# hlesmqh/WS3D

Hardware: AMD Instinct MI355X
Metric: KITTI scenes/sec (16384 pts) Stage-1 RPN fwd, 1/2/4/8 GPU; FPS+group HBM GB/s (higher is better)
Workload: dtype f32

## Files before the change

include/ws3d_ops.h:

```cpp
#ifndef WS3D_OPS_H
#define WS3D_OPS_H

#include <stddef.h>
#include <stdint.h>

#ifdef __cplusplus
extern "C" {
#endif

#define WS3D_OK 0
#define WS3D_E_INVALID (-1)
#define WS3D_E_LAUNCH (-2)
#define WS3D_E_WORKSPACE (-3)
#define WS3D_E_UNSUPPORTED (-4)

#if defined(__GNUC__)
#define WS3D_API __attribute__((visibility("default")))
#else
#define WS3D_API
#endif

typedef void *ws3d_stream_t;

#define WS3D_ABI_VERSION 6
// ... 162 lines not shown
                                const int32_t *idx, const float *weight, float *grad_points,
                                ws3d_stream_t stream);

WS3D_API size_t ws3d_scatter_workspace_bytes(int b, int c, int n_targets, long slots_per_scene);
WS3D_API int ws3d_group_points_grad_det(int b, int c, int n, int npoints, int nsample, const float *grad_out,
                                        const int32_t *idx, float *grad_points, void *workspace,
                                        size_t workspace_bytes, ws3d_stream_t stream);
WS3D_API int ws3d_three_interpolate_grad_det(int b, int c, int n, int m, const float *grad_out, const int32_t *idx,
                                             const float *weight, float *grad_points, void *workspace,
                                             size_t workspace_bytes, ws3d_stream_t stream);

WS3D_API int ws3d_bias_act_inplace(int b, int o_ch, long l, int relu, float *y, const float *bias,
                                   ws3d_stream_t stream);

WS3D_API int ws3d_rowmax_bias_act(int b, int o_ch, long m, int s, int relu, const float *y, const float *bias,
                                  float *out, ws3d_stream_t stream);

WS3D_API int ws3d_query_and_group_nlc(int b, int n, int m, int c, float radius, int nsample, int use_xyz,
                                      const float *xyz, const float *new_xyz, const float *features_nlc,
                                      int32_t *idx_out, float *out_nlc, const void *sorted, ws3d_stream_t stream);
WS3D_API int ws3d_three_interpolate_nlc(int b, int c, int m, int n, const float *feats_nlc, const int32_t *idx,
                                        const float *weight, float *out_nlc, int out_stride, ws3d_stream_t stream);
WS3D_API int ws3d_rowmax_rows(long rows_out, int ns, int o_ch, const float *y, float *out, int out_stride,
                              ws3d_stream_t stream);

WS3D_API int ws3d_sa_mlp3_pool(long rows, int nsample, int c1, int c2, int c3, const float *x_rows4,
                               const float *w1t, const float *b1, const float *w2t, const float *b2,
                               const float *w3t, const float *b3, int relu3, float *out, int out_stride,
                               ws3d_stream_t stream);

WS3D_API int ws3d_mlp2_rows(long rows, int k_dim, int o1, int o2, const float *x_rows, const float *w1t, const float *b1, int relu1,
                   const float *w2t, const float *b2, int relu2, float *out, int *ticket, ws3d_stream_t stream);

WS3D_API int ws3d_qinterp_gemm(int b, int n, int m, int c, int o_dim, const float *q, const int32_t *idx, const float *weight, const float *lin,
                      const float *skip, int c1, const float *wb, const float *b1, int relu1, const float *w2t, const float *b2, int relu2,
                      float *out, ws3d_stream_t stream);


WS3D_API int ws3d_boxes_overlap_bev(int num_a, const float *boxes_a, int num_b, const float *boxes_b,
                           float *ans, ws3d_stream_t stream);

WS3D_API int ws3d_boxes_iou_bev(int num_a, const float *boxes_a, int num_b, const float *boxes_b,
                       float *ans, ws3d_stream_t stream);

WS3D_API int ws3d_nms_mask(int boxes_num, const float *boxes, float thresh, int normal, int full_grid,
                  uint64_t *mask, ws3d_stream_t stream);

WS3D_API size_t ws3d_nms_workspace_bytes(int boxes_num);
WS3D_API int ws3d_nms(int boxes_num, const float *boxes, float thresh, int normal, int max_keep,
                      void *workspace, size_t workspace_bytes, int64_t *keep, int32_t *num_keep,
                      ws3d_stream_t stream);

WS3D_API int ws3d_nms_batched(int batch, int boxes_num, const float *boxes, float thresh, int normal,
                              int max_keep, void *workspace, size_t workspace_bytes, int64_t *keep,
                              int32_t *num_keep, ws3d_stream_t stream);


WS3D_API int ws3d_radius_nms_batched(int batch, int n, const float *centers, float radius, int max_keep,
                                     void *workspace, size_t workspace_bytes, int64_t *keep,
                                     int32_t *num_keep, ws3d_stream_t stream);

WS3D_API int ws3d_topk_sorted(int b, int n, int k, const float *scores, float *out_scores, int64_t *out_idx,
                              ws3d_stream_t stream);
WS3D_API size_t ws3d_topk_workspace_bytes(int b, int n);
WS3D_API int ws3d_topk_sorted_ws(int b, int n, int k, const float *scores, float *out_scores, int64_t *out_idx, void *workspace,
                                 size_t workspace_bytes, ws3d_stream_t stream);
// ... 67 lines not shown
```

ws3d_amd/_lib.py:

```python
from __future__ import annotations

import ctypes as C
import os

_HERE = os.path.dirname(os.path.abspath(__file__))
DIST_MODE = int(os.environ.get("WS3D_DIST_MODE", "0") or 0)
LIB_PATH = os.environ.get("WS3D_HIP_LIB") or os.path.join(
    _HERE, "libws3d_hip.so" if DIST_MODE == 0 else "libws3d_hip_dm%d.so" % DIST_MODE)

E_INVALID, E_LAUNCH, E_WORKSPACE, E_UNSUPPORTED = -1, -2, -3, -4
ABI_VERSION = 6

_vp = C.c_void_p
_i = C.c_int
_f = C.c_float
_sz = C.c_size_t

class CompactMlpArgs(C.Structure):
    _fields_ = [("b", _i), ("n", _i), ("m", _i), ("max_rows", C.c_long), ("o1", _i), ("o2", _i), ("o3", _i), ("pmat", _vp), ("p_stride", _i),
                ("xyz", _vp), ("new_xyz", _vp), ("rowc", _vp), ("rowsrc", _vp), ("total", _vp), ("w1x", _vp), ("b1", _vp), ("relu1", _i),
                ("w2t", _vp), ("b2", _vp), ("relu2", _i), ("w3t", _vp), ("b3", _vp), ("mid", _vp), ("out", _vp), ("out_stride", _i), ("limit", C.c_long)]


SIGNATURES = {
# ... 11 lines not shown
    "ws3d_ball_query": (_i, [_i, _i, _i, _f, _i, _vp, _vp, _vp, _vp, _vp]),
    "ws3d_ball_query_fill": (_i, [_i, _i, _i, _f, _i, _vp, _vp, _vp, _vp, _vp]),
    "ws3d_ball_query_pairs": (_i, [_i, _i, _i, _f, _i, _vp, _vp, _vp, _vp, _vp, _vp, _vp, _vp]),
    "ws3d_ball_query_pairs2": (_i, [_i, _i, _i, _vp, _vp, _vp, C.c_float, _i, _vp, _vp, _vp, _vp, C.c_float, _i, _vp, _vp, _vp, _vp, _vp]),
    "ws3d_sorted_points_bytes": (_sz, [_i, _i]),
    "ws3d_sort_points_x": (_i, [_i, _i, _vp, _vp, _vp]),
    "ws3d_sort_points_xz": (_i, [_i, _i, _vp, _vp, _vp]),
    "ws3d_sort_points_grid": (_i, [_i, _i, _vp, _vp, _vp]),
    "ws3d_sort_points_jobs": (_i, [_i, _i, _vp, _vp, _vp, _vp, _vp]),
    "ws3d_group_points": (_i, [_i, _i, _i, _i, _i, _vp, _vp, _vp, _vp]),
    "ws3d_group_points_grad": (_i, [_i, _i, _i, _i, _i, _vp, _vp, _vp, _vp]),
    "ws3d_query_and_group": (_i, [_i, _i, _i, _i, _f, _i, _i, _vp, _vp, _vp, _vp, _vp, _vp, _vp]),
    "ws3d_three_nn": (_i, [_i, _i, _i, _vp, _vp, _vp, _vp, _vp, _vp]),
    "ws3d_three_interpolate": (_i, [_i, _i, _i, _i, _vp, _vp, _vp, _vp, _vp]),
    "ws3d_three_interpolate_grad": (_i, [_i, _i, _i, _i, _vp, _vp, _vp, _vp, _vp]),
    "ws3d_bn_workspace_bytes": (C.c_size_t, [_i, _i, C.c_long]),
    "ws3d_bn_relu_train_fwd": (_i, [_i, _i, C.c_long, _vp, _vp, _vp, C.c_float, C.c_float, _i, _vp, _vp, _vp, _vp, _vp, _vp,
                                    _vp, C.c_size_t, _vp]),
    "ws3d_bn_relu_train_bwd": (_i, [_i, _i, C.c_long, _vp, _vp, _vp, _vp, _vp, _vp, _i, _vp, _vp, _vp, _vp, C.c_size_t, _vp]),
    "ws3d_conv1x1_wgrad_workspace_bytes": (C.c_size_t, [_i, _i, _i, C.c_long]),
    "ws3d_conv1x1_wgrad": (_i, [_i, _i, _i, C.c_long, _vp, _vp, _vp, _vp, C.c_size_t, _vp]),
    "ws3d_gemm_pool": (_i, [C.c_long, _i, _i, _i, _vp, _vp, _vp, _i, _vp, _i, _vp, C.c_long, _vp]),
    "ws3d_pool_nsample": (_i, [C.c_long, _i, _vp, _vp, _vp, _vp]),
    "ws3d_pool_nsample_grad": (_i, [C.c_long, _i, _vp, _vp, _vp, _vp]),
    "ws3d_scatter_workspace_bytes": (C.c_size_t, [_i, _i, _i, C.c_long]),
    "ws3d_group_points_grad_det": (_i, [_i, _i, _i, _i, _i, _vp, _vp, _vp, _vp, C.c_size_t, _vp]),
    "ws3d_three_interpolate_grad_det": (_i, [_i, _i, _i, _i, _vp, _vp, _vp, _vp, _vp, C.c_size_t, _vp]),
    "ws3d_query_and_group_nlc": (_i, [_i, _i, _i, _i, _f, _i, _i, _vp, _vp, _vp, _vp, _vp, _vp, _vp]),
    "ws3d_three_interpolate_nlc": (_i, [_i, _i, _i, _i, _vp, _vp, _vp, _vp, _i, _vp]),
    "ws3d_rowmax_rows": (_i, [C.c_long, _i, _i, _vp, _vp, _i, _vp]),
    "ws3d_sa_mlp3_pool": (_i, [C.c_long, _i, _i, _i, _i, _vp, _vp, _vp, _vp, _vp, _vp, _vp, _i, _vp, _i, _vp]),
    "ws3d_qinterp_gemm": (_i, [_i, _i, _i, _i, _i, _vp, _vp, _vp, _vp, _vp, _i, _vp, _vp, _i, _vp, _vp, _i, _vp, _vp]),
    "ws3d_mlp2_rows": (_i, [C.c_long, _i, _i, _i, _vp, _vp, _vp, _i, _vp, _vp, _i, _vp, _vp, _vp]),
    "ws3d_decode_center_boxes": (_i, [_i, _i, _i, _f, _f, _f, _f, _f, _vp, _vp, _vp, _vp]),
    "ws3d_topk_sorted": (_i, [_i, _i, _i, _vp, _vp, _vp, _vp]),
    "ws3d_topk_workspace_bytes": (C.c_size_t, [_i, _i]),
    "ws3d_topk_sorted_ws": (_i, [_i, _i, _i, _vp, _vp, _vp, _vp, C.c_size_t, _vp]),
    "ws3d_topk_sorted_sigmoid": (_i, [_i, _i, _i, _vp, _vp, _vp, _vp]),
    "ws3d_topk_sorted_sigmoid_ws": (_i, [_i, _i, _i, _vp, _vp, _vp, _vp, C.c_size_t, _vp]),
    "ws3d_three_nn_weights": (_i, [C.c_long, _vp, _vp, _vp]),
    "ws3d_three_nn_w": (_i, [_i, _i, _i, _vp, _vp, _vp, _vp, _vp, _vp, _vp]),
    "ws3d_three_nn_wq": (_i, [_i, _i, _i, _vp, _vp, _vp, _vp, _vp, _vp, _vp, _vp]),
    "ws3d_three_nn_jobs": (_i, [_i, _i, _vp, _vp, _vp, _vp, _vp, _vp, _vp, _vp, _vp]),
    "ws3d_bias_act_inplace": (_i, [_i, _i, C.c_long, _i, _vp, _vp, _vp]),
    "ws3d_rowmax_bias_act": (_i, [_i, _i, C.c_long, _i, _i, _vp, _vp, _vp, _vp]),
    "ws3d_boxes_overlap_bev": (_i, [_i, _vp, _i, _vp, _vp, _vp]),
    "ws3d_boxes_iou_bev": (_i, [_i, _vp, _i, _vp, _vp, _vp]),
    "ws3d_nms_mask": (_i, [_i, _vp, _f, _i, _i, _vp, _vp]),
    "ws3d_nms_workspace_bytes": (_sz, [_i]),
    "ws3d_nms": (_i, [_i, _vp, _f, _i, _i, _vp, _sz, _vp, _vp, _vp]),
    "ws3d_nms_batched": (_i, [_i, _i, _vp, _f, _i, _i, _vp, _sz, _vp, _vp, _vp]),
    "ws3d_radius_nms_batched": (_i, [_i, _i, _vp, _f, _i, _vp, _sz, _vp, _vp, _vp]),
    "ws3d_gather_gemm": (_i, [_i, _i, _i, _i, _i, _i, _vp, _vp, _vp, _vp, _vp, _vp, _i, _vp, _vp]),
    "ws3d_gather_gemm2": (_i, [_i, _i, _i, _i, _i, _i, _i, _vp, _vp, _vp, _vp, _vp, _vp, _i, _vp, _vp, _i, _vp, _vp]),
    "ws3d_pgather_gemm2": (_i, [_i, _i, _i, _i, _i, _i, _vp, _i, _vp, _vp, _vp, _vp, _vp, _i, _vp, _vp, _i, _vp, _vp, C.c_long, _vp]),
    "ws3d_pgather_rows": (_i, [_i, _i, _i, _i, _i, _vp, _i, _vp, _vp, _vp, _vp, _vp, _i, _vp, _vp]),
    "ws3d_qinterp_rows": (_i, [_i, _i, _i, _i, _vp, _vp, _vp, _vp, _vp, _i, _vp, _vp, _i, _vp, _vp]),
    "ws3d_compact_pairs": (_i, [C.c_long, _i, _vp, _vp, _vp, _vp, _vp]),
    "ws3d_compact_pairs_count": (_i, [C.c_long, _i, _vp, _vp, _vp]),
    "ws3d_compact_pairs_rows": (_i, [C.c_long, _i, _vp, _vp, _vp, _vp, _vp, _vp, _vp]),
    "ws3d_pgather_gemm2_compact": (_i, [_i, _i, _i, C.c_long, _i, _i, _vp, _i, _vp, _vp, _vp, _vp, _vp, _vp, _vp, _i, _vp, _vp, _i, _vp, C.c_long, _vp]),
    "ws3d_pgather_gemm3_compact": (_i, [_i, _i, _i, C.c_long, _i, _i, _i, _vp, _i, _vp, _vp, _vp, _vp, _vp, _vp, _vp, _i, _vp, _vp, _i, _vp, _vp, _vp, _i, C.c_long, _vp]),
    "ws3d_gemm_pool_compact": (_i, [C.c_long, _i, _i, _vp, _vp, _vp, _vp, _vp, _vp, _i, C.c_long, _vp]),
    "ws3d_compact_mlp_pair": (_i, [_i, C.POINTER(CompactMlpArgs), C.POINTER(CompactMlpArgs), _vp]),
    "ws3d_chain_mlp3_ticket_ints": (_i, []),
    "ws3d_chain_mlp3_blob_floats": (_sz, [_i]),
# ... 62 lines not shown
```

ws3d_amd/build.py:

```python
from __future__ import annotations

import argparse
import concurrent.futures as cf
import os
import shutil
import subprocess
import sys

HERE = os.path.dirname(os.path.abspath(__file__))
CSRC = os.path.join(HERE, "csrc")
OBJ = os.path.join(CSRC, "build")
LIB = os.path.join(HERE, "libws3d_hip.so")
DIST_MODES = (0, 1, 2)


def lib_path(dist_mode: int = 0) -> str:
    return LIB if dist_mode == 0 else os.path.join(HERE, "libws3d_hip_dm%d.so" % dist_mode)
ARCH = "gfx950"
SOURCES = ["core.hip", "fps.hip", "fps_v3.hip", "fps_bucket.hip", "fps_nested.hip", "ballquery_group.hip", "interpolate.hip", "roipool3d.hip", "iou3d.hip", "proposals.hip", "scatter_det.hip", "sa_mlp.hip", "bn_relu.hip", "gemm_pool.hip", "conv_wgrad.hip", "chain_mlp.hip", "kitti_eval.hip"]
CXXFLAGS = ["-O3", "-std=c++17", "-fPIC", "-ffp-contract=off", "-fno-fast-math",
            "-fvisibility=hidden", "-Wall", "-Wno-unused-function"]


def hipcc() -> str:
    for cand in (os.environ.get("HIPCC"), shutil.which("hipcc"), "/opt/rocm/bin/hipcc"):
        if cand and os.path.exists(cand):
            return cand
    raise RuntimeError("hipcc not found (looked at $HIPCC, PATH, /opt/rocm/bin)")


def _deps(src: str):
    return [src, os.path.join(CSRC, "common.h"), os.path.join(CSRC, "binning.h"), os.path.join(CSRC, "compact_pool.h"), os.path.join(HERE, "..", "include", "ws3d_ops.h"),
            os.path.join(CSRC, "exports.map"), os.path.abspath(__file__)]


def _compile(src: str, force: bool, verbose: bool, dist_mode: int = 0) -> str:
    path = os.path.join(CSRC, src)
    obj = os.path.join(OBJ if dist_mode == 0 else OBJ + "_dm%d" % dist_mode, os.path.splitext(src)[0] + ".o")
    if not force and os.path.exists(obj) and all(
            os.path.getmtime(obj) >= os.path.getmtime(d) for d in _deps(path)):
        return obj
    cmd = [hipcc(), f"--offload-arch={ARCH}", *CXXFLAGS, f"-DWS3D_DIST_MODE={dist_mode}", *os.environ.get("WS3D_EXTRA_DEFS", "").split(), "-c", path, "-o", obj]
    if verbose:
        print(" ".join(cmd), flush=True)
    r = subprocess.run(cmd, capture_output=True, text=True)
    if r.returncode != 0:
        raise RuntimeError(f"hipcc failed for {src}:\n{r.stdout}\n{r.stderr}")
    if verbose and r.stderr.strip():
        print(r.stderr)
    return obj


# ... 43 lines not shown
```

ws3d_amd/compat.py:

```python
from __future__ import annotations

import sys
import types

import os

import torch

from . import _lib
from ._lib import Ws3dError, check


def _dev(*tensors):
    dev = None
    for t in tensors:
        if t is None:
            continue
        if not t.is_cuda:
            raise Ws3dError("ws3d_amd ops need HIP ('cuda') tensors; there is no CPU fallback")
        if not t.is_contiguous():
            raise Ws3dError("ws3d_amd ops need contiguous tensors (the reference asserts the same)")
        if dev is None:
            dev = t.device
        elif t.device != dev:
# ... 715 lines not shown
    _f32(known_feats, "known_feats"); _i32(idx, "idx"); _f32(weight, "weight"); _f32(wt, "wt")
    B, M, C2 = known_feats.shape
    N = idx.size(1)
    C1 = 0 if unknown_feats is None else unknown_feats.size(2)
    O = wt.size(1)
    rows = B * N
    if (C2 % 4 or O % 64 or rows % 64 or rows // 64 > 65535 or wt.size(0) != C2 + C1 or not known_feats.is_contiguous() or
            (unknown_feats is not None and not unknown_feats.is_contiguous())):
        return None
    out = torch.empty((rows, O), dtype=torch.float32, device=dev)
    with _on(dev):
        check(_lib.load().ws3d_interp_gemm(B, N, M, C2, C1, O, _p(known_feats), _p(unknown_feats), _p(idx), _p(weight), _p(wt), _p(bias),
                                           int(bool(relu)), _p(out), _stream()), "interp_gemm")
    return out


def mlp2_rows(x2d, w1t, b1, relu1, w2t, b2, relu2, ticket=None):
    dev = _dev(x2d, w1t, w2t)
    _f32(x2d, "x2d"); _f32(w1t, "w1t"); _f32(w2t, "w2t")
    R, K = x2d.shape
    O1, O2 = w1t.size(1), w2t.size(1)
    if (K != 128 or O1 != 128 or w1t.size(0) != 128 or w2t.size(0) != 128 or O2 > 64 or R % 32 or not x2d.is_contiguous() or
            not w1t.is_contiguous() or not w2t.is_contiguous()):
        return None
    out = torch.empty((R, O2), dtype=torch.float32, device=dev)
    if ticket is None:
        ticket = torch.zeros(1, dtype=torch.int32, device=dev)
    with _on(dev):
        check(_lib.load().ws3d_mlp2_rows(R, K, O1, O2, _p(x2d), _p(w1t), _p(b1), int(bool(relu1)), _p(w2t), _p(b2), int(bool(relu2)),
                                         _p(out), _p(ticket), _stream()), "mlp2_rows")
    return out


def pool_nsample(x):
    dev = _dev(x)
    _f32(x, "x")
    ns = x.size(-1)
    out = torch.empty(x.shape[:-1], dtype=torch.float32, device=dev)
    arg = torch.empty(x.shape[:-1], dtype=torch.uint8, device=dev)
    with _on(dev):
        check(_lib.load().ws3d_pool_nsample(out.numel(), ns, _p(x), _p(out), _p(arg), _stream()), "pool_nsample")
    return out, arg


def pool_nsample_grad(grad_out, arg, nsample):
    dev = _dev(grad_out, arg)
    _f32(grad_out, "grad_out")
    if arg.dtype != torch.uint8 or not arg.is_contiguous():
        raise TypeError("arg must be a contiguous uint8 tensor")
    grad_x = torch.empty(tuple(grad_out.shape) + (nsample,), dtype=torch.float32, device=dev)
    with _on(dev):
        check(_lib.load().ws3d_pool_nsample_grad(grad_out.numel(), nsample, _p(grad_out), _p(arg), _p(grad_x), _stream()),
              "pool_nsample_grad")
    return grad_x


SA_MLP3_SHAPES = {(16, 16, 32), (32, 32, 64)}


def sa_mlp3_pool(x_rows4, nsample, layers, out, col0=0):
    (w1, b1, r1), (w2, b2, r2), (w3, b3, r3) = layers
    widths = (w1.size(1), w2.size(1), w3.size(1))
    if (x_rows4.size(1) != 4 or widths not in SA_MLP3_SHAPES or nsample not in (16, 32) or not (r1 and r2)
            or b1 is None or b2 is None or b3 is None):
        return False
    dev = _dev(x_rows4, out)
# ... 425 lines not shown
```

ws3d_amd/fastpath.py:

```python
from __future__ import annotations

import contextlib
import contextvars

import torch
import torch.nn as nn

from . import compat as _C
from . import nn_blocks, pn2_ops

FUSED_SA_MLP = True
SA1_FROM_LISTS = True
FUSED_GEMM_POOL = True
FUSED_INTERP_GEMM = True
NESTED_FPS = True
GEOMETRY_AHEAD = True
_AHEAD_OVERRIDE = contextvars.ContextVar("ws3d_geometry_ahead", default=None)


@contextlib.contextmanager
def geometry_ahead(on: bool):
    token = _AHEAD_OVERRIDE.set(bool(on))
    try:
        yield
# ... 8 lines not shown
        yield
    finally:
        _COMPACT_ONLY.reset(token)


def primed_compact_scales(net, pointcloud: torch.Tensor, margin: float = None):
    margin = PRIMED_MARGIN if margin is None else margin
    keys, per_level = set(), {}
    for row in list_fill(net, pointcloud):
        si = per_level.get(row["level"], 0)
        per_level[row["level"]] = si + 1
        if row["fill"] <= margin * COMPACT_MAX_FILL:
            keys.add((row["level"] - 1, si))
    return frozenset(keys)


def _geometry_ahead_now() -> bool:
    v = _AHEAD_OVERRIDE.get()
    return GEOMETRY_AHEAD if v is None else v
GEOMETRY_IN_CAPTURE = False
PER_POINT_L1 = True
COMPACT_MAX_FILL = 0.55
COMPACT_PAIRS = True
PAIR_DISPATCH = "device"
PRIMED_MARGIN = 0.85
_COMPACT_ONLY = contextvars.ContextVar("ws3d_compact_only_scales", default=frozenset())
CHAIN_MLP = True
PAIRED_SCALES = True
MERGED_THREE_NN = True
FUSED_PROLOGUE = True
MERGED_BINNING = True
PER_POINT_FP = True
FUSED_MLP2_ROWS = True
FUSED_GATHER_GEMM2 = True
BIN_INPUT_AHEAD = True
FUSED_QINTERP_GEMM_MIN_ROWS = 30000
FUSED_COMPACT3_MAX_LDS = 64 * 1024
FUSED_GATHER_GEMM = True
GRID_MIN_N = 256
DUAL_SCALE_SEARCH = True
NESTED_CHAIN = True
QUERY_CELL_ORDER = True
PARALLEL_SCALES = True
PARALLEL_HEADS = True


def _row_weights(block):
    w, shift, act = block._folded()
    if act is not None and not isinstance(act, nn.ReLU):
        raise NotImplementedError("fast path supports ReLU / no activation only")
    cache = block.__dict__.get("_row_cache")
    if cache is None or cache[0] is not w:
        cache = (w, w.t().contiguous())
        if not torch.cuda.is_current_stream_capturing():
            block.__dict__["_row_cache"] = cache
    return cache[1], shift, act is not None


def _row_weights_xyz_last(block):
    wt, bias, relu = _row_weights(block)
    cache = block.__dict__.get("_row_cache_xyz_last")
    if cache is None or cache[0] is not wt:
        cache = (wt, torch.cat((wt[3:], wt[:3]), dim=0).contiguous())
        if not torch.cuda.is_current_stream_capturing():
            block.__dict__["_row_cache_xyz_last"] = cache
    return cache[1], bias, relu
# ... 2 lines not shown
def _split_rows(block, wt: torch.Tensor, c2: int):
    cache = block.__dict__.get("_split_cache")
    if cache is None or cache[0] is not wt or cache[1] != c2:
        cache = (wt, c2, wt[:c2].contiguous(), wt[c2:].contiguous())
        if not torch.cuda.is_current_stream_capturing():
            block.__dict__["_split_cache"] = cache
    return cache[2], cache[3]


def _layer(x2d: torch.Tensor, block) -> torch.Tensor:
    wt, bias, relu = _row_weights(block)
    if bias is None:
        y = torch.mm(x2d, wt)
        return torch.relu_(y) if relu else y
    if relu:
        return torch._addmm_activation(bias, x2d, wt, use_gelu=False)
    return torch.addmm(bias, x2d, wt)


def _blocks(seq):
    return [m for m in seq if isinstance(m, nn_blocks._ConvBlock)]


def mlp_rows(x2d: torch.Tensor, seq, ticket=None) -> torch.Tensor:
    blocks = _blocks(seq)
    if FUSED_MLP2_ROWS and len(blocks) == 2 and x2d.size(1) == 128 and x2d.is_contiguous():
        (w1, b1, r1), (w2, b2, r2) = _row_weights(blocks[0]), _row_weights(blocks[1])
        y = _C.mlp2_rows(x2d, w1, b1, r1, w2, b2, r2, ticket)
        if y is not None:
            return y
    for blk in blocks:
        x2d = _layer(x2d, blk)
    return x2d


def supported(model) -> bool:
    try:
        for m in model.modules():
            if isinstance(m, nn_blocks._ConvBlock):
                if not m._pointwise or not isinstance(getattr(m, "activation", None), (nn.ReLU, type(None))):
                    return False
        for sa in model.rpn.backbone_net.SA_modules:
            if sa.pool_method != "max_pool" or sa.npoint is None:
                return False
            for g, mlp in zip(sa.groupers, sa.mlps):
                if not isinstance(g, pn2_ops.QueryAndGroup) or any(b.conv.out_channels % 4 for b in _blocks(mlp)):
                    return False
        return True
    except AttributeError:
        return False


def _gather_gemm_ok(sa, grouper, blocks, c_feat: int, B: int) -> bool:
    return (FUSED_GATHER_GEMM and c_feat >= 16 and c_feat % 4 == 0 and grouper.use_xyz and len(blocks) >= 2 and
            blocks[0].conv.out_channels % 64 == 0 and (B * sa.npoint * grouper.nsample) % 64 == 0 and
            (B * sa.npoint * grouper.nsample) // 64 <= 65535)


def _pair_limit(rows: int, dense_available: bool, key=None) -> int:
    if PAIR_DISPATCH != "device" or not dense_available or (key is not None and key in _COMPACT_ONLY.get()):
        return -1
    return max(0, int(COMPACT_MAX_FILL * rows))


@torch.no_grad()
def list_fill(net, pointcloud: torch.Tensor):
# ... 443 lines not shown
                    if _C.BQ_FINE_GRID:
                        pre_grid = {k + 1: ((next(bufs),) if x_.size(1) >= GRID_MIN_N else (None,)) for k, x_ in enumerate(lv[:-1])}
                        pre_xz = {k + 1: (next(bufs) if x_.size(1) >= 256 else None) for k, x_ in enumerate(lv)}
                        if MERGED_THREE_NN:
                            allx = [l_xyz[0]] + lv
                            qgrid = {0: binned[0]}
                            qgrid.update({k_: v_[0] for k_, v_ in pre_grid.items()})
                            lvls = [k_ for k_ in range(len(sas)) if pre_xz.get(k_ + 1) is not None and allx[k_ + 1].size(1) <= 4096]
                            got = _C.three_nn_jobs([(allx[k_], allx[k_ + 1], pre_xz[k_ + 1], qgrid.get(k_) if QUERY_CELL_ORDER else None) for k_ in lvls])
                            if got is not None:
                                nn_pre = dict(zip(lvls, got))
        for i in range(-1, -(len(net.FP_modules) + 1), -1):
            lvl = len(l_xyz) + i - 1
            nn3 = nn_pre.get(lvl)
            if geo is not None:
                geo.main.wait_event(geo.nn_ready[lvl])
                nn3 = geo.nn[lvl]
            known_level = len(l_xyz) + i
            l_feats[i - 1] = fp_forward(net.FP_modules[i], l_xyz[i - 1], l_xyz[i], l_feats[i - 1], l_feats[i], nn3, binned[len(l_xyz) + i - 1],
                                        (pre_xz[known_level],) if known_level in pre_xz else None)
    finally:
        if geo is not None:
            geo.release()
    return l_xyz[0], l_feats[0]


@torch.no_grad()
def rpn_forward(model, pts_input: torch.Tensor, defer_reg_join: bool = False) -> dict:
    rpn = model.rpn
    zeros = _arena_for(rpn.backbone_net, pts_input.size(0), pts_input.device, extra=8, clear=not FUSED_PROLOGUE)
    xyz, feats = backbone_forward(rpn.backbone_net, pts_input, zeros)
    B, N, C = feats.shape
    rows = feats.view(B * N, C)
    tickets = zeros.take((2,), torch.int32) if FUSED_MLP2_ROWS else (None, None)
    reg_ready = None
    if PARALLEL_HEADS and _geometry_ahead_now() and not torch.cuda.is_current_stream_capturing():
        main = torch.cuda.current_stream(rows.device)
        aux = _side_streams(main)[2]
        fork = torch.cuda.Event()
        fork.record(main)
        aux.wait_event(fork)
        with torch.cuda.stream(aux):
            rpn_reg = mlp_rows(rows, rpn.rpn_reg_layer, tickets[1:2]).view(B, N, -1)
            reg_ready = torch.cuda.Event()
            reg_ready.record(aux)
        rpn_reg.record_stream(main)
        rpn_cls = mlp_rows(rows, rpn.rpn_cls_layer, tickets[0:1]).view(B, N, -1)
        if not defer_reg_join:
            main.wait_event(reg_ready)
            reg_ready = None
    else:
        rpn_cls = mlp_rows(rows, rpn.rpn_cls_layer, tickets[0:1]).view(B, N, -1)
        rpn_reg = mlp_rows(rows, rpn.rpn_reg_layer, tickets[1:2]).view(B, N, -1)
    global LAST_ARENA_FALLBACKS
    LAST_ARENA_FALLBACKS = zeros.fallbacks if not zeros.fallbacks else getattr(zeros, "fallback_shapes", zeros.fallbacks)
    out = {"rpn_cls": rpn_cls, "rpn_reg": rpn_reg, "backbone_xyz": xyz,
           "backbone_features": feats.transpose(1, 2),
           "backbone_features_nlc": feats}
    if reg_ready is not None:
        out["rpn_reg_ready"] = reg_ready
    return out
```

ws3d_amd/pipeline.py:

```python
from __future__ import annotations

import os
from typing import Iterable, Iterator, Tuple

import numpy as np
import torch

from . import roipool3d_ops, stage1


def ensure_hw_queues(n: int = 32) -> bool:
    if torch.cuda.is_initialized():
        return False
    os.environ.setdefault("GPU_MAX_HW_QUEUES", str(n))
    return True


def _hw_queue_cap() -> int:
    try:
        return int(os.environ.get("GPU_MAX_HW_QUEUES", "4"))
    except ValueError:
        return 4


# ... 99 lines not shown

    def _prime(self, slot: dict) -> None:
        slot["primed"] = True
        if not self.use_graph or self.graph_error is not None:
            return
        prev = self._tunable(True)
        try:
            with _LaunchGeometry(self.depth >= THROUGHPUT_GEOMETRY_MIN_DEPTH):
                self._prime_capture(slot)
        finally:
            if prev is not None:
                torch.cuda.tunable.enable(prev[0])
                torch.cuda.tunable.tuning_enable(prev[1])

    def _prime_capture(self, slot: dict) -> None:
        try:
            stream = slot["stream"]
            stream.wait_stream(torch.cuda.current_stream(self.device))
            from . import fastpath
            if self.compact_only is None:
                with torch.cuda.stream(stream):
                    blank = not bool(slot["inp"].any().item())
                    self.compact_only = (fastpath.primed_compact_scales(self.model.rpn.backbone_net, slot["inp"])
                                         if (self.pair_dispatch == "primed" and not blank) else frozenset())
                    self.compact_only_source = "blank input: both forms kept" if blank else ("fills of the first primed batch" if self.pair_dispatch == "primed" else "pair_dispatch=device")
            with fastpath.geometry_ahead(False), fastpath.compact_only_scales(self.compact_only), torch.cuda.stream(stream):
                for _ in range(2):
                    self.body(slot["inp"], slot["exchange"])
            stream.synchronize()
            graph = torch.cuda.CUDAGraph()
            with fastpath.compact_only_scales(self.compact_only), torch.cuda.graph(graph, stream=stream):
                slot["out"] = self.body(slot["inp"], slot["exchange"])
            slot["graph"] = graph
        except Exception as exc:
            self.graph_error = repr(exc)
            slot["graph"] = None

    def capture_all(self) -> bool:
        for slot in self.slots:
            if not slot["primed"]:
                slot["inp"].copy_(self.slots[0]["inp"])
                self._prime(slot)
        torch.cuda.synchronize(self.device)
        return self.use_graph and self.graph_error is None

    @torch.no_grad()
    def submit(self, pts=None) -> int:
        slot = self.slots[self.submitted % self.depth]
        with torch.cuda.device(self.device):
            if pts is not None:
                t = torch.from_numpy(np.ascontiguousarray(pts, dtype=np.float32)) if not torch.is_tensor(pts) else pts
                if t.size(0) > self.B or tuple(t.shape[1:]) != tuple(slot["inp"].shape[1:]):
                    raise ValueError(f"batch of shape {tuple(t.shape)} does not fit the pipeline's {tuple(slot['inp'].shape)}")
            if not slot["primed"]:
                if pts is not None:
                    slot["inp"][:t.size(0)].copy_(t)
                    if t.size(0) < self.B:
                        slot["inp"][t.size(0):] = slot["inp"][t.size(0) - 1]
                self._prime(slot)
            if pts is not None and t.is_cuda:
                slot["stream"].wait_stream(torch.cuda.current_stream(self.device))
                t.record_stream(slot["stream"])
            with torch.cuda.stream(slot["stream"]):
                if pts is not None:
                    slot["inp"][:t.size(0)].copy_(t, non_blocking=True)
                    if t.size(0) < self.B:
# ... 33 lines not shown
```

Baseline: 6463.

## Add fused RPN cls/reg head kernel using split-bf16 MFMA with LDS-resident weights

Adds a new HIP kernel that computes the RPN classification and regression two-layer heads in one launch. Weights are prepacked once into a cached blob as three-way bf16 splits, and activations are split the same way on the fly so 6-term MFMA products approximate f32 accuracy. Workgroups are divided between the cls and reg heads and pull 32-row tiles dynamically through atomic tickets. The aim is to replace the per-head mlp_rows launches and their scalar FP32 math with matrix-core throughput and one shared pass over the feature rows. The risks are the extra MFMA work from the bf16 splitting, small numeric differences from f32, and blob caching that must be kept alive across graph capture.

```diff
diff --git a/include/ws3d_ops.h b/include/ws3d_ops.h
--- a/include/ws3d_ops.h
+++ b/include/ws3d_ops.h
@@ -218,6 +218,12 @@
 WS3D_API int ws3d_mlp2_rows(long rows, int k_dim, int o1, int o2, const float *x_rows, const float *w1t, const float *b1, int relu1,
                    const float *w2t, const float *b2, int relu2, float *out, int *ticket, ws3d_stream_t stream);
 
+WS3D_API size_t ws3d_rpn_heads_blob_bytes(int o2);
+WS3D_API int ws3d_rpn_heads_pack(int o2, const float *w1t, const float *b1, int relu1, const float *w2t, const float *b2, int relu2, void *blob,
+                        ws3d_stream_t stream);
+WS3D_API int ws3d_rpn_heads(long rows, const float *x_rows, int heads, const void *blob_cls, float *out_cls, int *ticket_cls, int o2_reg,
+                   const void *blob_reg, float *out_reg, int *ticket_reg, int workgroups, ws3d_stream_t stream);
+
 WS3D_API int ws3d_qinterp_gemm(int b, int n, int m, int c, int o_dim, const float *q, const int32_t *idx, const float *weight, const float *lin,
                       const float *skip, int c1, const float *wb, const float *b1, int relu1, const float *w2t, const float *b2, int relu2,
                       float *out, ws3d_stream_t stream);
diff --git a/ws3d_amd/_lib.py b/ws3d_amd/_lib.py
--- a/ws3d_amd/_lib.py
+++ b/ws3d_amd/_lib.py
@@ -67,6 +67,9 @@
     "ws3d_sa_mlp3_pool": (_i, [C.c_long, _i, _i, _i, _i, _vp, _vp, _vp, _vp, _vp, _vp, _vp, _i, _vp, _i, _vp]),
     "ws3d_qinterp_gemm": (_i, [_i, _i, _i, _i, _i, _vp, _vp, _vp, _vp, _vp, _i, _vp, _vp, _i, _vp, _vp, _i, _vp, _vp]),
     "ws3d_mlp2_rows": (_i, [C.c_long, _i, _i, _i, _vp, _vp, _vp, _i, _vp, _vp, _i, _vp, _vp, _vp]),
+    "ws3d_rpn_heads_blob_bytes": (_sz, [_i]),
+    "ws3d_rpn_heads_pack": (_i, [_i, _vp, _vp, _i, _vp, _vp, _i, _vp, _vp]),
+    "ws3d_rpn_heads": (_i, [C.c_long, _vp, _i, _vp, _vp, _vp, _i, _vp, _vp, _vp, _i, _vp]),
     "ws3d_decode_center_boxes": (_i, [_i, _i, _i, _f, _f, _f, _f, _f, _vp, _vp, _vp, _vp]),
     "ws3d_topk_sorted": (_i, [_i, _i, _i, _vp, _vp, _vp, _vp]),
     "ws3d_topk_workspace_bytes": (C.c_size_t, [_i, _i]),
diff --git a/ws3d_amd/build.py b/ws3d_amd/build.py
--- a/ws3d_amd/build.py
+++ b/ws3d_amd/build.py
@@ -17,7 +17,7 @@
 def lib_path(dist_mode: int = 0) -> str:
     return LIB if dist_mode == 0 else os.path.join(HERE, "libws3d_hip_dm%d.so" % dist_mode)
 ARCH = "gfx950"
-SOURCES = ["core.hip", "fps.hip", "fps_v3.hip", "fps_bucket.hip", "fps_nested.hip", "ballquery_group.hip", "interpolate.hip", "roipool3d.hip", "iou3d.hip", "proposals.hip", "scatter_det.hip", "sa_mlp.hip", "bn_relu.hip", "gemm_pool.hip", "conv_wgrad.hip", "chain_mlp.hip", "kitti_eval.hip"]
+SOURCES = ["core.hip", "fps.hip", "fps_v3.hip", "fps_bucket.hip", "fps_nested.hip", "ballquery_group.hip", "interpolate.hip", "roipool3d.hip", "iou3d.hip", "proposals.hip", "scatter_det.hip", "sa_mlp.hip", "bn_relu.hip", "gemm_pool.hip", "conv_wgrad.hip", "chain_mlp.hip", "rpn_heads.hip", "kitti_eval.hip"]
 CXXFLAGS = ["-O3", "-std=c++17", "-fPIC", "-ffp-contract=off", "-fno-fast-math",
             "-fvisibility=hidden", "-Wall", "-Wno-unused-function"]
 
diff --git a/ws3d_amd/compat.py b/ws3d_amd/compat.py
--- a/ws3d_amd/compat.py
+++ b/ws3d_amd/compat.py
@@ -771,6 +771,44 @@
     return out
 
 
+def rpn_heads_pack(w1t, b1, relu1, w2t, b2, relu2):
+    dev = _dev(w1t, w2t)
+    _f32(w1t, "w1t"); _f32(w2t, "w2t")
+    O2 = w2t.size(1) if w2t.dim() == 2 else 0
+    n = int(_lib.load().ws3d_rpn_heads_blob_bytes(O2))
+    if n == 0 or tuple(w1t.shape) != (128, 128) or w2t.size(0) != 128 or not w1t.is_contiguous() or not w2t.is_contiguous():
+        return None
+    for b, nm, o in ((b1, "b1", 128), (b2, "b2", O2)):
+        if b is not None:
+            _f32(b, nm)
+            if b.numel() != o or not b.is_contiguous():
+                return None
+    blob = torch.empty((n + 15) // 16 * 4, dtype=torch.float32, device=dev)
+    with _on(dev):
+        check(_lib.load().ws3d_rpn_heads_pack(O2, _p(w1t), _p(b1), int(bool(relu1)), _p(w2t), _p(b2), int(bool(relu2)), _p(blob), _stream()),
+              "rpn_heads_pack")
+    return blob
+
+
+def rpn_heads(x2d, heads, blob_cls, blob_reg, o2_reg, tickets, workgroups=0):
+    dev = _dev(x2d)
+    _f32(x2d, "x2d")
+    if (x2d.dim() != 2 or x2d.size(1) != 128 or x2d.size(0) % 32 or not x2d.is_contiguous() or heads not in (1, 2, 3) or
+            tickets is None or tickets.dtype != torch.int32 or tickets.numel() < 2 or not tickets.is_contiguous()):
+        return None
+    R = x2d.size(0)
+    out_cls = torch.empty((R, 1), dtype=torch.float32, device=dev) if heads & 1 else None
+    out_reg = torch.empty((R, int(o2_reg)), dtype=torch.float32, device=dev) if heads & 2 else None
+    with _on(dev):
+        rc = _lib.load().ws3d_rpn_heads(R, _p(x2d), int(heads), _p(blob_cls) if heads & 1 else None, _p(out_cls), _p(tickets[0:1]),
+                                        int(o2_reg) if heads & 2 else 0, _p(blob_reg) if heads & 2 else None, _p(out_reg), _p(tickets[1:2]),
+                                        int(workgroups), _stream())
+    if rc == _lib.E_UNSUPPORTED:
+        return None
+    check(rc, "rpn_heads")
+    return out_cls, out_reg
+
+
 def pool_nsample(x):
     dev = _dev(x)
     _f32(x, "x")
diff --git a/ws3d_amd/csrc/rpn_heads.hip b/ws3d_amd/csrc/rpn_heads.hip
--- /dev/null
+++ b/ws3d_amd/csrc/rpn_heads.hip
@@ -0,0 +1,291 @@
+#include <algorithm>
+
+#include "common.h"
+
+namespace ws3d {
+
+typedef float heads_f16 __attribute__((ext_vector_type(16)));
+typedef __bf16 heads_bf8 __attribute__((ext_vector_type(8)));
+
+constexpr int HEADS_K = 128;
+constexpr int HEADS_KS = HEADS_K + 8;
+constexpr int HEADS_THREADS = 512;
+constexpr int HEADS_MAX_O2 = 64;
+
+constexpr int HB_W1P = 16;
+constexpr int HB_B1 = HB_W1P + 3 * HEADS_K * HEADS_KS * 2;
+constexpr int HB_B2 = HB_B1 + 4 * HEADS_K;
+constexpr int HB_W2 = HB_B2 + 4 * HEADS_MAX_O2;
+__host__ __device__ constexpr int heads_blob_bytes(int o2) { return HB_W2 + (o2 == 1 ? 4 * HEADS_K : 3 * o2 * HEADS_KS * 2); }
+static_assert(HB_W2 % 16 == 0 && heads_blob_bytes(HEADS_MAX_O2) <= 160 * 1024, "rpn_heads blob layout");
+
+__device__ __forceinline__ void heads_split3(float x, __bf16 &p1, __bf16 &p2, __bf16 &p3) {
+    p1 = (__bf16)x;
+    const float r1 = x - (float)p1;
+    p2 = (__bf16)r1;
+    const float r2 = r1 - (float)p2;
+    p3 = (__bf16)r2;
+}
+
+__device__ __forceinline__ void heads_split8(const float *v, heads_bf8 &q1, heads_bf8 &q2, heads_bf8 &q3) {
+#pragma unroll
+    for (int j = 0; j < 8; ++j) {
+        __bf16 p1, p2, p3;
+        heads_split3(v[j], p1, p2, p3);
+        q1[j] = p1; q2[j] = p2; q3[j] = p3;
+    }
+}
+
+__device__ __forceinline__ heads_f16 heads_mfma6(const heads_bf8 &w1, const heads_bf8 &w2, const heads_bf8 &w3, const heads_bf8 &b1,
+                                                 const heads_bf8 &b2, const heads_bf8 &b3, heads_f16 c) {
+    c = __builtin_amdgcn_mfma_f32_32x32x16_bf16(w3, b1, c, 0, 0, 0);
+    c = __builtin_amdgcn_mfma_f32_32x32x16_bf16(w2, b2, c, 0, 0, 0);
+    c = __builtin_amdgcn_mfma_f32_32x32x16_bf16(w1, b3, c, 0, 0, 0);
+    c = __builtin_amdgcn_mfma_f32_32x32x16_bf16(w2, b1, c, 0, 0, 0);
+    c = __builtin_amdgcn_mfma_f32_32x32x16_bf16(w1, b2, c, 0, 0, 0);
+    c = __builtin_amdgcn_mfma_f32_32x32x16_bf16(w1, b1, c, 0, 0, 0);
+    return c;
+}
+
+__device__ __forceinline__ float heads_relu(float y) { return y < 0.f ? 0.f : y; }
+
+__host__ __device__ constexpr int heads_w2_channel(int kk) {
+    return (kk & ~31) + 16 * ((kk >> 4) & 1) + 8 * ((kk & 7) >> 2) + 4 * ((kk >> 3) & 1) + (kk & 3);
+}
+
+__global__ __launch_bounds__(256) void rpn_heads_pack_kernel(int o2, const float *__restrict__ w1t, const float *__restrict__ b1, int relu1,
+                                                             const float *__restrict__ w2t, const float *__restrict__ b2, int relu2,
+                                                             unsigned char *__restrict__ blob) {
+    const int t = blockIdx.x * blockDim.x + threadIdx.x, nt = gridDim.x * blockDim.x;
+    if (t == 0) {
+        int *hdr = reinterpret_cast<int *>(blob);
+        hdr[0] = o2; hdr[1] = relu1; hdr[2] = relu2; hdr[3] = 0;
+    }
+    __bf16 *w1p = reinterpret_cast<__bf16 *>(blob + HB_W1P);
+    for (int i = t; i < HEADS_K * HEADS_KS; i += nt) {
+        const int o = i / HEADS_KS, k = i - o * HEADS_KS;
+        __bf16 p1, p2, p3;
+        heads_split3(k < HEADS_K ? w1t[k * HEADS_K + o] : 0.f, p1, p2, p3);
+        w1p[i] = p1; w1p[HEADS_K * HEADS_KS + i] = p2; w1p[2 * HEADS_K * HEADS_KS + i] = p3;
+    }
+    float *bb1 = reinterpret_cast<float *>(blob + HB_B1), *bb2 = reinterpret_cast<float *>(blob + HB_B2);
+    for (int i = t; i < HEADS_K; i += nt) bb1[i] = b1 ? b1[i] : 0.f;
+    for (int i = t; i < HEADS_MAX_O2; i += nt) bb2[i] = (b2 && i < o2) ? b2[i] : 0.f;
+    if (o2 == 1) {
+        float *w2 = reinterpret_cast<float *>(blob + HB_W2);
+        for (int i = t; i < HEADS_K; i += nt) w2[i] = w2t[i];
+    } else {
+        __bf16 *w2p = reinterpret_cast<__bf16 *>(blob + HB_W2);
+        for (int i = t; i < o2 * HEADS_KS; i += nt) {
+            const int o = i / HEADS_KS, kk = i - o * HEADS_KS;
+            __bf16 p1, p2, p3;
+            heads_split3(kk < HEADS_K ? w2t[heads_w2_channel(kk) * o2 + o] : 0.f, p1, p2, p3);
+            w2p[i] = p1; w2p[o2 * HEADS_KS + i] = p2; w2p[2 * o2 * HEADS_KS + i] = p3;
+        }
+    }
+}
+
+template <int NB2>
+__device__ __forceinline__ void rpn_head_walk(long tiles, const float *__restrict__ x, const unsigned char *lds, float *__restrict__ out,
+                                              int *__restrict__ ticket, int *next_chunk, long chunk) {
+    const int tid = threadIdx.x, lane = tid & 63, r = lane & 31, h = lane >> 5;
+    const int *hdr = reinterpret_cast<const int *>(lds);
+    const int o2 = hdr[0], relu1 = hdr[1], relu2 = hdr[2];
+    const __bf16 *w1p = reinterpret_cast<const __bf16 *>(lds + HB_W1P) + r * HEADS_KS + 8 * h;
+    const float *b1s = reinterpret_cast<const float *>(lds + HB_B1), *b2s = reinterpret_cast<const float *>(lds + HB_B2);
+    constexpr int PIECE1 = HEADS_K * HEADS_KS;
+    for (int par = 0; chunk * 8 < tiles; par ^= 1) {
+        int ahead = 0;
+        if (tid == 0) ahead = atomicAdd(ticket, 1);
+        const long tile = chunk * 8 + (tid >> 6);
+        if (tile < tiles) {
+            float xv[64];
+            const float4 *xp = reinterpret_cast<const float4 *>(x + (tile * 32 + r) * HEADS_K + 8 * h);
+#pragma unroll
+            for (int s = 0; s < 8; ++s) {
+                const float4 t0 = xp[4 * s], t1 = xp[4 * s + 1];
+                xv[8 * s] = t0.x; xv[8 * s + 1] = t0.y; xv[8 * s + 2] = t0.z; xv[8 * s + 3] = t0.w;
+                xv[8 * s + 4] = t1.x; xv[8 * s + 5] = t1.y; xv[8 * s + 6] = t1.z; xv[8 * s + 7] = t1.w;
+            }
+            heads_f16 acc[4];
+#pragma unroll
+            for (int blk = 0; blk < 4; ++blk)
+#pragma unroll
+                for (int i = 0; i < 16; ++i) acc[blk][i] = 0.f;
+#pragma unroll
+            for (int s = 0; s < 8; ++s) {
+                heads_bf8 q1, q2, q3;
+                heads_split8(xv + 8 * s, q1, q2, q3);
+#pragma unroll
+                for (int blk = 0; blk < 4; ++blk) {
+                    const __bf16 *wr = w1p + blk * 32 * HEADS_KS + 16 * s;
+                    const heads_bf8 a1 = *reinterpret_cast<const heads_bf8 *>(wr);
+                    const heads_bf8 a2 = *reinterpret_cast<const heads_bf8 *>(wr + PIECE1);
+                    const heads_bf8 a3 = *reinterpret_cast<const heads_bf8 *>(wr + 2 * PIECE1);
+                    acc[blk] = heads_mfma6(a1, a2, a3, q1, q2, q3, acc[blk]);
+                }
+            }
+#pragma unroll
+            for (int blk = 0; blk < 4; ++blk)
+#pragma unroll
+                for (int v = 0; v < 16; ++v) {
+                    const float y = acc[blk][v] + b1s[blk * 32 + (v & 3) + 8 * (v >> 2) + 4 * h];
+                    acc[blk][v] = relu1 ? heads_relu(y) : y;
+                }
+            if constexpr (NB2 == 0) {
+                const float *w2s = reinterpret_cast<const float *>(lds + HB_W2);
+                float p = 0.f;
+#pragma unroll
+                for (int blk = 0; blk < 4; ++blk)
+#pragma unroll
+                    for (int v = 0; v < 16; ++v) p = __builtin_fmaf(acc[blk][v], w2s[blk * 32 + (v & 3) + 8 * (v >> 2) + 4 * h], p);
+                const float q = __shfl_xor(p, 32);
+                float y = (h ? q + p : p + q) + b2s[0];
+                if (relu2) y = heads_relu(y);
+                if (h == 0) out[tile * 32 + r] = y;
+            } else {
+                const __bf16 *w2p = reinterpret_cast<const __bf16 *>(lds + HB_W2);
+                const int piece2 = o2 * HEADS_KS;
+                heads_f16 y[NB2];
+#pragma unroll
+                for (int ob = 0; ob < NB2; ++ob)
+#pragma unroll
+                    for (int i = 0; i < 16; ++i) y[ob][i] = 0.f;
+#pragma unroll
+                for (int blk = 0; blk < 4; ++blk)
+#pragma unroll
+                    for (int s = 0; s < 2; ++s) {
+                        heads_bf8 q1, q2, q3;
+                        float av[8];
+#pragma unroll
+                        for (int j = 0; j < 8; ++j) av[j] = acc[blk][8 * s + j];
+                        heads_split8(av, q1, q2, q3);
+#pragma unroll
+                        for (int ob = 0; ob < NB2; ++ob) {
+                            const int o = min(ob * 32 + r, o2 - 1);
+                            const __bf16 *wr = w2p + o * HEADS_KS + blk * 32 + 16 * s + 8 * h;
+                            const heads_bf8 a1 = *reinterpret_cast<const heads_bf8 *>(wr);
+                            const heads_bf8 a2 = *reinterpret_cast<const heads_bf8 *>(wr + piece2);
+                            const heads_bf8 a3 = *reinterpret_cast<const heads_bf8 *>(wr + 2 * piece2);
+                            y[ob] = heads_mfma6(a1, a2, a3, q1, q2, q3, y[ob]);
+                        }
+                    }
+                float *orow = out + (tile * 32 + r) * (long)o2;
+#pragma unroll
+                for (int ob = 0; ob < NB2; ++ob)
+#pragma unroll
+                    for (int g = 0; g < 4; ++g) {
+                        const int o0 = ob * 32 + 8 * g + 4 * h;
+                        if (o0 < o2) {
+                            float v4[4];
+#pragma unroll
+                            for (int e = 0; e < 4; ++e) {
+                                v4[e] = y[ob][4 * g + e] + b2s[o0 + e];
+                                if (relu2) v4[e] = heads_relu(v4[e]);
+                            }
+                            if (o2 % 4 == 0) {
+                                *reinterpret_cast<float4 *>(orow + o0) = make_float4(v4[0], v4[1], v4[2], v4[3]);
+                            } else {
+#pragma unroll
+                                for (int e = 0; e < 4; ++e)
+                                    if (o0 + e < o2) orow[o0 + e] = v4[e];
+                            }
+                        }
+                    }
+            }
+        }
+        if (tid == 0) next_chunk[par ^ 1] = ahead;
+        __syncthreads();
+        chunk = next_chunk[par ^ 1];
+    }
+}
+
+template <int NB2>
+__global__ __launch_bounds__(HEADS_THREADS) void rpn_heads_kernel(long tiles, const float *__restrict__ x, int wg_cls,
+                                                                  const unsigned char *__restrict__ blob_cls, float *__restrict__ out_cls,
+                                                                  int *__restrict__ ticket_cls, const unsigned char *__restrict__ blob_reg,
+                                                                  float *__restrict__ out_reg, int *__restrict__ ticket_reg, int o2_reg) {
+    extern __shared__ __attribute__((aligned(16))) unsigned char smem_heads[];
+    __shared__ int next_chunk[2];
+    const bool cls = (int)blockIdx.x < wg_cls;
+    const unsigned char *blob = cls ? blob_cls : blob_reg;
+    int *ticket = cls ? ticket_cls : ticket_reg;
+    const int tid = threadIdx.x;
+    if (tid == 0) next_chunk[0] = atomicAdd(ticket, 1);
+    const int n16 = heads_blob_bytes(cls ? 1 : o2_reg) / 16;
+    for (int i = tid; i < n16; i += HEADS_THREADS) reinterpret_cast<uint4 *>(smem_heads)[i] = reinterpret_cast<const uint4 *>(blob)[i];
+    __syncthreads();
+    const long chunk = next_chunk[0];
+    if (cls)
+        rpn_head_walk<0>(tiles, x, smem_heads, out_cls, ticket, next_chunk, chunk);
+    else
+        rpn_head_walk<NB2>(tiles, x, smem_heads, out_reg, ticket, next_chunk, chunk);
+}
+
+static int heads_cu_count() {
+    static int cus[64] = {0};
+    int dev = 0;
+    if (hipGetDevice(&dev) != hipSuccess || dev < 0 || dev >= 64) dev = 0;
+    if (cus[dev] == 0) {
+        int n = 0;
+        if (hipDeviceGetAttribute(&n, hipDeviceAttributeMultiprocessorCount, dev) != hipSuccess || n <= 0) n = 256;
+        cus[dev] = n;
+    }
+    return cus[dev];
+}
+
+}
+
+extern "C" size_t ws3d_rpn_heads_blob_bytes(int o2) {
+    return (o2 >= 1 && o2 <= ws3d::HEADS_MAX_O2) ? (size_t)ws3d::heads_blob_bytes(o2) : 0;
+}
+
+extern "C" int ws3d_rpn_heads_pack(int o2, const float *w1t, const float *b1, int relu1, const float *w2t, const float *b2, int relu2, void *blob,
+                                   ws3d_stream_t stream) {
+    using namespace ws3d;
+    if (!w1t || !w2t || !blob || (reinterpret_cast<uintptr_t>(blob) & 15)) { set_error("ws3d_rpn_heads_pack: invalid argument"); return WS3D_E_INVALID; }
+    if (ws3d_rpn_heads_blob_bytes(o2) == 0) {
+        set_error("ws3d_rpn_heads_pack: unsupported o2 = %d (1 .. %d)", o2, HEADS_MAX_O2);
+        return WS3D_E_UNSUPPORTED;
+    }
+    hipLaunchKernelGGL(rpn_heads_pack_kernel, dim3(64), dim3(256), 0, as_stream(stream), o2, w1t, b1, relu1 ? 1 : 0, w2t, b2, relu2 ? 1 : 0,
+                       static_cast<unsigned char *>(blob));
+    return check_launch("ws3d_rpn_heads_pack");
+}
+
+extern "C" int ws3d_rpn_heads(long rows, const float *x_rows, int heads, const void *blob_cls, float *out_cls, int *ticket_cls, int o2_reg,
+                              const void *blob_reg, float *out_reg, int *ticket_reg, int workgroups, ws3d_stream_t stream) {
+    using namespace ws3d;
+    const bool do_cls = heads & 1, do_reg = heads & 2;
+    const uintptr_t al = reinterpret_cast<uintptr_t>(x_rows) | reinterpret_cast<uintptr_t>(do_cls ? blob_cls : nullptr) |
+                         reinterpret_cast<uintptr_t>(do_reg ? blob_reg : nullptr) | reinterpret_cast<uintptr_t>(do_reg && o2_reg % 4 == 0 ? out_reg : nullptr);
+    if (rows < 0 || (heads & ~3) || !heads || !x_rows || (al & 15) || (do_cls && (!blob_cls || !out_cls || !ticket_cls)) ||
+        (do_reg && (!blob_reg || !out_reg || !ticket_reg))) {
+        set_error("ws3d_rpn_heads: invalid argument (rows=%ld heads=%d)", rows, heads);
+        return WS3D_E_INVALID;
+    }
+    if ((rows & 31) || (do_reg && ws3d_rpn_heads_blob_bytes(o2_reg) == 0) || (do_reg && o2_reg == 1)) {
+        set_error("ws3d_rpn_heads: unsupported shape (rows=%ld o2=%d; rows %% 32, 2 <= o2 <= %d)", rows, o2_reg, HEADS_MAX_O2);
+        return WS3D_E_UNSUPPORTED;
+    }
+    if (rows == 0) return WS3D_OK;
+    const long tiles = rows / 32, chunks = (tiles + 7) / 8;
+    const long wgs_all = workgroups > 0 ? workgroups : heads_cu_count();
+    long wg_cls = 0, wg_reg = 0;
+    if (do_cls && do_reg) {
+        wg_cls = std::max(1L, std::min(chunks, (wgs_all * 2 + 2) / 5));
+        wg_reg = std::max(1L, std::min(chunks, wgs_all - wg_cls));
+    } else {
+        (do_cls ? wg_cls : wg_reg) = std::max(1L, std::min(chunks, wgs_all));
+    }
+    const size_t lds = (size_t)std::max(heads_blob_bytes(1), do_reg ? heads_blob_bytes(o2_reg) : 0);
+    auto go = [&](auto kern) -> int {
+        if (int rc = raise_lds_cap((const void *)kern, lds, "ws3d_rpn_heads")) return rc;
+        hipLaunchKernelGGL(kern, dim3((unsigned)(wg_cls + wg_reg)), dim3(HEADS_THREADS), lds, as_stream(stream), tiles, x_rows, (int)wg_cls,
+                           static_cast<const unsigned char *>(blob_cls), out_cls, ticket_cls, static_cast<const unsigned char *>(blob_reg), out_reg,
+                           ticket_reg, o2_reg);
+        return WS3D_OK;
+    };
+    if (int rc = (do_reg && o2_reg > 32) ? go(rpn_heads_kernel<2>) : go(rpn_heads_kernel<1>)) return rc;
+    return check_launch("ws3d_rpn_heads");
+}
diff --git a/ws3d_amd/fastpath.py b/ws3d_amd/fastpath.py
--- a/ws3d_amd/fastpath.py
+++ b/ws3d_amd/fastpath.py
@@ -64,6 +64,7 @@
 MERGED_BINNING = True
 PER_POINT_FP = True
 FUSED_MLP2_ROWS = True
+FUSED_HEADS = True
 FUSED_GATHER_GEMM2 = True
 BIN_INPUT_AHEAD = True
 FUSED_QINTERP_GEMM_MIN_ROWS = 30000
@@ -132,6 +133,33 @@
     for blk in blocks:
         x2d = _layer(x2d, blk)
     return x2d
+
+
+def _heads_blob(seq):
+    blocks = _blocks(seq)
+    if len(blocks) != 2:
+        return None
+    (w1, b1, r1), (w2, b2, r2) = _row_weights(blocks[0]), _row_weights(blocks[1])
+    cache = blocks[0].__dict__.get("_heads_blob")
+    if cache is None or cache[0] is not w1 or cache[1] is not b1 or cache[2] is not w2 or cache[3] is not b2:
+        cache = (w1, b1, w2, b2, _C.rpn_heads_pack(w1, b1, r1, w2, b2, r2), w2.size(1))
+        if not torch.cuda.is_current_stream_capturing():
+            blocks[0].__dict__["_heads_blob"] = cache
+    return None if cache[4] is None else (cache[4], cache[5])
+
+
+def heads_blobs(rpn):
+    return [blk.__dict__["_heads_blob"][4] for seq in (rpn.rpn_cls_layer, rpn.rpn_reg_layer) for blk in _blocks(seq)[:1]
+            if "_heads_blob" in blk.__dict__]
+
+
+def _fused_heads(rows: torch.Tensor, blobs, which: int, tickets):
+    if blobs is None or not all(blobs[i] is not None for i in (0, 1) if which & (1 << i)):
+        return None
+    (bc, oc), (br, orr) = blobs[0] or (None, 1), blobs[1] or (None, 0)
+    if oc != 1 or (which & 2 and orr == 1):
+        return None
+    return _C.rpn_heads(rows, which, bc, br, orr, tickets, _C.tune("mlp2_wgs") * (2 if which == 3 else 1))
 
 
 def supported(model) -> bool:
@@ -641,7 +669,8 @@
     xyz, feats = backbone_forward(rpn.backbone_net, pts_input, zeros)
     B, N, C = feats.shape
     rows = feats.view(B * N, C)
-    tickets = zeros.take((2,), torch.int32) if FUSED_MLP2_ROWS else (None, None)
+    tickets = zeros.take((2,), torch.int32) if (FUSED_MLP2_ROWS or FUSED_HEADS) else (None, None)
+    blobs = (_heads_blob(rpn.rpn_cls_layer), _heads_blob(rpn.rpn_reg_layer)) if FUSED_HEADS else None
     reg_ready = None
     if PARALLEL_HEADS and _geometry_ahead_now() and not torch.cuda.is_current_stream_capturing():
         main = torch.cuda.current_stream(rows.device)
@@ -650,17 +679,23 @@
         fork.record(main)
         aux.wait_event(fork)
         with torch.cuda.stream(aux):
-            rpn_reg = mlp_rows(rows, rpn.rpn_reg_layer, tickets[1:2]).view(B, N, -1)
+            fused = _fused_heads(rows, blobs, 2, tickets)
+            rpn_reg = (fused[1] if fused is not None else mlp_rows(rows, rpn.rpn_reg_layer, tickets[1:2])).view(B, N, -1)
             reg_ready = torch.cuda.Event()
             reg_ready.record(aux)
         rpn_reg.record_stream(main)
-        rpn_cls = mlp_rows(rows, rpn.rpn_cls_layer, tickets[0:1]).view(B, N, -1)
+        fused = _fused_heads(rows, blobs, 1, tickets)
+        rpn_cls = (fused[0] if fused is not None else mlp_rows(rows, rpn.rpn_cls_layer, tickets[0:1])).view(B, N, -1)
         if not defer_reg_join:
             main.wait_event(reg_ready)
             reg_ready = None
     else:
-        rpn_cls = mlp_rows(rows, rpn.rpn_cls_layer, tickets[0:1]).view(B, N, -1)
-        rpn_reg = mlp_rows(rows, rpn.rpn_reg_layer, tickets[1:2]).view(B, N, -1)
+        fused = _fused_heads(rows, blobs, 3, tickets)
+        if fused is not None:
+            rpn_cls, rpn_reg = fused[0].view(B, N, -1), fused[1].view(B, N, -1)
+        else:
+            rpn_cls = mlp_rows(rows, rpn.rpn_cls_layer, tickets[0:1]).view(B, N, -1)
+            rpn_reg = mlp_rows(rows, rpn.rpn_reg_layer, tickets[1:2]).view(B, N, -1)
     global LAST_ARENA_FALLBACKS
     LAST_ARENA_FALLBACKS = zeros.fallbacks if not zeros.fallbacks else getattr(zeros, "fallback_shapes", zeros.fallbacks)
     out = {"rpn_cls": rpn_cls, "rpn_reg": rpn_reg, "backbone_xyz": xyz,
diff --git a/ws3d_amd/pipeline.py b/ws3d_amd/pipeline.py
--- a/ws3d_amd/pipeline.py
+++ b/ws3d_amd/pipeline.py
@@ -155,6 +155,7 @@
             with fastpath.compact_only_scales(self.compact_only), torch.cuda.graph(graph, stream=stream):
                 slot["out"] = self.body(slot["inp"], slot["exchange"])
             slot["graph"] = graph
+            slot["heads_blobs"] = fastpath.heads_blobs(self.model.rpn)
         except Exception as exc:
             self.graph_error = repr(exc)
             slot["graph"] = None
```

Result: faster. 6837, median of 6 (+5.8%).
